# kidusabe1/Imagined-Speech-Decoding

Hardware: AMD Instinct MI355X
Metric: trials/sec end-to-end (filterbank+CNN fwd+bwd) (higher is better)
Workload: dtype f32; 1 GPU; cfg2: 64ch x 2s@256Hz EEG, 9-band Butterworth(4) filterbank -> STFT(64/32) log band power -> Conv4Layers(576,32)+Linear(32,5) fwd+bwd, softmax-CE, AdamW; trials_per_gpu=4096, global_batch=4096, parallelism=dp1, streams=one stream

## Files before the change

imagined-speech-decoding_amd/csrc/conv.hip:

```cpp
#include "common.h"
#include <math.h>
#include <string.h>
#include <type_traits>
#include <vector>

namespace isd {

typedef float f32x2 __attribute__((ext_vector_type(2)));

constexpr int kTaps = 5;
constexpr int kCK = 32;
constexpr int kMaxZones = 64;

struct ZoneDesc {
  int cin;
  int idx_off;
  int64_t p_off;
  int64_t eff_off;
  int64_t wg_off;
};

struct bf16_t { unsigned short v; };
__device__ __forceinline__ float bf16_round(float x) {
  unsigned int u = __float_as_uint(x);
// ... 2609 lines not shown
    for (int ii = wave; ii < n_it; ii += 4) {
      float* dst = buf + ii * item_len;
      glds_copy16((const float*)a.dout + ((is + ii) * a.Z + z) * (int64_t)do_len, dst, do_len >> 2, lane);
      glds_copy16((const float*)a.in + ((is + ii) * a.Ctot + chan0 + c_base) * (int64_t)a.Tx, dst + do_len,
                  (cw * a.Tin) >> 2, lane);
    }
  };
  const unsigned smem_base = (unsigned)(uintptr_t)(__attribute__((address_space(3))) float*)smem;
  const int do_q = do_len >> 2, in_q = (cw * a.Tin) >> 2;
  const bool fast = a.IPS <= 4 && do_q <= kGldsRunMax4 && in_q <= kGldsRunMax4;
  const uint64_t do_tail = __builtin_amdgcn_ballot_w64(lane < (do_q & 63));
  const uint64_t in_tail = __builtin_amdgcn_ballot_w64(lane < (in_q & 63));
  const char* do_src = (const char*)a.dout + ((i_lo + wave_s) * a.Z + z) * (int64_t)do_len * 4;
  const char* in_src = (const char*)a.in + ((i_lo + wave_s) * a.Ctot + chan0 + c_base) * (int64_t)a.Tx * 4;
  const int64_t do_step = (int64_t)a.IPS * a.Z * do_len * 4, in_step = (int64_t)a.IPS * a.Ctot * a.Tx * 4;
  const unsigned slot_lds = smem_base + (unsigned)(wave_s * item_len) * 4;
  const unsigned lane16 = lane * 16;
  auto stage_fast = [&](int n_it, int s) {
    if (wave_s < n_it) {
      const unsigned dst = slot_lds + (unsigned)(s * buf_len) * 4;
      glds_run(do_q >> 6, do_tail, dst, do_src, lane16);
      glds_run(in_q >> 6, in_tail, dst + (unsigned)do_len * 4, in_src, lane16);
    }
    do_src += do_step;
    in_src += in_step;
  };

  f32x4 acc[GT][kTaps], accb[GT];
#pragma unroll
  for (int g = 0; g < GT; ++g) {
    accb[g] = (f32x4){0.f, 0.f, 0.f, 0.f};
#pragma unroll
    for (int k = 0; k < kTaps; ++k) acc[g][k] = (f32x4){0.f, 0.f, 0.f, 0.f};
  }
  struct Frag {
    float af[GT];
    float bf[kTaps];
    float one;
  };
  const int a_off = jl * a.Tout + q;
  const int b_off = do_len + (wave * 16 + jl) * a.Tin + q;
  struct FragSet {
    float af[GT];
    f32x2 b01, b23;
    float b4;
  };
  constexpr int kSetReads = GT + 3;
  const unsigned zero_addr = smem_base + (unsigned)(2 * buf_len) * 4;
  auto run_packed = [&](auto bias, int sbuf, int n_it) {
    const unsigned buf_addr = smem_base + (unsigned)(sbuf * buf_len) * 4;
    unsigned a0 = buf_addr + (unsigned)a_off * 4, a1 = a0 + (unsigned)(16 * a.Tout) * 4, b = buf_addr + (unsigned)b_off * 4;
    int p_ii = 0, p_t = q;
    const unsigned wrap = (unsigned)(item_len - a.Tout + 4) * 4;
    auto issue = [&](FragSet& f) {
      const bool dead = p_ii >= n_it;
      const unsigned ra0 = dead ? zero_addr : a0, ra1 = dead ? zero_addr : a1, rb = dead ? zero_addr : b;
      if constexpr (GT == 2)
        asm volatile("ds_read_b32 %0, %5\n\tds_read_b32 %1, %6\n\tds_read2_b32 %2, %7 offset1:1\n\t"
                     "ds_read2_b32 %3, %7 offset0:2 offset1:3\n\tds_read_b32 %4, %7 offset:16"
                     : "=&v"(f.af[0]), "=&v"(f.af[GT - 1]), "=&v"(f.b01), "=&v"(f.b23), "=&v"(f.b4)
                     : "v"(ra0), "v"(ra1), "v"(rb)
                     : "memory");
      else
        asm volatile("ds_read_b32 %0, %4\n\tds_read2_b32 %1, %5 offset1:1\n\t"
                     "ds_read2_b32 %2, %5 offset0:2 offset1:3\n\tds_read_b32 %3, %5 offset:16"
                     : "=&v"(f.af[0]), "=&v"(f.b01), "=&v"(f.b23), "=&v"(f.b4)
                     : "v"(ra0), "v"(rb)
                     : "memory");
      p_t += 4;
      const bool w = p_t >= a.Tout;
      const unsigned d = w ? wrap : 16u;
      a0 += d; a1 += d; b += d;
      if (w) { p_t -= a.Tout; ++p_ii; }
    };
    auto take = [&](FragSet& f, auto behind) {
      if constexpr (GT == 2)
        asm volatile("s_waitcnt lgkmcnt(%5)" : "+v"(f.af[0]), "+v"(f.af[GT - 1]), "+v"(f.b01), "+v"(f.b23), "+v"(f.b4)
                     : "i"(decltype(behind)::value) : "memory");
      else
        asm volatile("s_waitcnt lgkmcnt(%4)" : "+v"(f.af[0]), "+v"(f.b01), "+v"(f.b23), "+v"(f.b4)
                     : "i"(decltype(behind)::value) : "memory");
      __builtin_amdgcn_sched_barrier(0);
    };
    auto mma_set = [&](const FragSet& f) {
      const float bf[kTaps] = {f.b01[0], f.b01[1], f.b23[0], f.b23[1], f.b4};
#pragma unroll
      for (int k = 0; k < kTaps; ++k)
#pragma unroll
        for (int g = 0; g < GT; ++g) acc[g][k] = __builtin_amdgcn_mfma_f32_16x16x4f32(f.af[g], bf[k], acc[g][k], 0, 0, 0);
      if constexpr (decltype(bias)::value) {
#pragma unroll
        for (int g = 0; g < GT; ++g) accb[g] = __builtin_amdgcn_mfma_f32_16x16x4f32(f.af[g], 1.f, accb[g], 0, 0, 0);
      }
      __builtin_amdgcn_sched_barrier(0);
    };
    const int n_step = (n_it * a.Tout + 3) >> 2;
    const std::integral_constant<int, kSetReads> one_set;
    const std::integral_constant<int, 0> none;
    FragSet f0, f1;
    issue(f0);
    int st = 1;
    for (; st + 1 < n_step; st += 2) {
      issue(f1);
      take(f0, one_set);
      mma_set(f0);
      issue(f0);
      take(f1, one_set);
      mma_set(f1);
    }
    if (st < n_step) {
      issue(f1);
      take(f0, one_set);
      mma_set(f0);
      take(f1, none);
      mma_set(f1);
    } else {
      take(f0, none);
      mma_set(f0);
    }
  };
  auto run_single = [&](int sbuf, int n_it) {
    const float* buf = smem + sbuf * buf_len;
    auto load = [&](int ii, Frag& f) {
      const bool ok = q < a.Tout;
      const float* ib = buf + ii * item_len;
#pragma unroll
      for (int g = 0; g < GT; ++g) {
        const float v = ib[a_off + g * 16 * a.Tout];
        f.af[g] = ok ? v : 0.f;
      }
#pragma unroll
      for (int k = 0; k < kTaps; ++k) {
        const float v = ib[b_off + k];
        f.bf[k] = ok ? v : 0.f;
      }
      f.one = ok ? 1.f : 0.f;
    };
    auto mma = [&](const Frag& f) {
#pragma unroll
      for (int k = 0; k < kTaps; ++k)
#pragma unroll
        for (int g = 0; g < GT; ++g) acc[g][k] = __builtin_amdgcn_mfma_f32_16x16x4f32(f.af[g], f.bf[k], acc[g][k], 0, 0, 0);
      if (with_bias) {
#pragma unroll
        for (int g = 0; g < GT; ++g) accb[g] = __builtin_amdgcn_mfma_f32_16x16x4f32(f.af[g], f.one, accb[g], 0, 0, 0);
      }
    };
    Frag f0, f1;
    load(0, f0);
    for (int st = 0; st < n_it; st += 2) {
      if (st + 1 < n_it) load(st + 1, f1);
      mma(f0);
      if (st + 1 < n_it) {
// ... 172 lines not shown

static int conv5_wgrad_wide_bf16_item_floats(int F, int W) { return (16 * F / 2 + 64 * W + 3) & ~3; }

struct ReduceDst {
  float *o0, *o1, *o2;
  int64_t n0, n1;
};
__global__ __launch_bounds__(256) void reduce_slabs_kernel(float* __restrict__ part, ReduceDst out,
                                                           int64_t n, int n_slabs, int L, int stride) {
  __shared__ float red[4][64];
  const int lane = threadIdx.x & 63, grp = threadIdx.x >> 6;
  const int64_t e = (int64_t)blockIdx.x * 64 + lane;
  const int k0 = blockIdx.y * L;
  const int k1 = k0 + L < n_slabs ? k0 + L : n_slabs;
  float s0 = 0.f, s1 = 0.f;
  if (e < n) {
    int k = k0 + grp;
    for (; k + 4 < k1; k += 8) {
      s0 += part[(int64_t)k * stride * n + e];
      s1 += part[(int64_t)(k + 4) * stride * n + e];
    }
    if (k < k1) s0 += part[(int64_t)k * stride * n + e];
  }
  red[grp][lane] = s0 + s1;
  __syncthreads();
  if (grp == 0 && e < n) {
    const float v = (red[0][lane] + red[1][lane]) + (red[2][lane] + red[3][lane]);
    if (gridDim.y > 1) part[(int64_t)k0 * stride * n + e] = v;
    else if (e < out.n0) out.o0[e] = v;
    else if (e < out.n0 + out.n1) out.o1[e - out.n0] = v;
    else out.o2[e - out.n0 - out.n1] = v;
  }
}

static inline void launch_reduce_slabs(float* part, ReduceDst out, int64_t n, int n_slabs, hipStream_t st) {
  const unsigned bx = (unsigned)cdiv(n, 64);
  if (n_slabs >= 64 && bx < 1024) {
    int L = 8;
    while (L * L < n_slabs) L *= 2;
    const int S = (int)cdiv(n_slabs, L);
    hipLaunchKernelGGL(reduce_slabs_kernel, dim3(bx, S), dim3(256), 0, st, part, out, n, n_slabs, L, 1);
    hipLaunchKernelGGL(reduce_slabs_kernel, dim3(bx, 1), dim3(256), 0, st, part, out, n, S, S, L);
  } else {
    hipLaunchKernelGGL(reduce_slabs_kernel, dim3(bx, 1), dim3(256), 0, st, part, out, n, n_slabs, n_slabs, 1);
  }
}
static inline void launch_reduce_slabs(float* part, float* out, int64_t n, int n_slabs, hipStream_t st) {
  launch_reduce_slabs(part, ReduceDst{out, nullptr, nullptr, n, 0}, n, n_slabs, st);
}

struct SlabJob {
  float* part;
  float* out;
  int64_t n;
  int n_slabs, L;
  int layer;
  unsigned bx0;
};
struct SlabJobs {
  SlabJob j[3];
  const ZoneDesc* zones;
  int F;
};
__global__ __launch_bounds__(256) void reduce_jobs_kernel(SlabJobs js, int level) {
  __shared__ float red[4][64];
  const int ji = blockIdx.x >= js.j[2].bx0 ? 2 : (blockIdx.x >= js.j[1].bx0 ? 1 : 0);
  const SlabJob jb = js.j[ji];
  const int lane = threadIdx.x & 63, grp = threadIdx.x >> 6;
  const int64_t e = (int64_t)(blockIdx.x - jb.bx0) * 64 + lane, n = jb.n;
  const int two = jb.L < jb.n_slabs;
  int k0, k1, stride;
  if (level == 2) {
    if (!two) return;
    k0 = 0; k1 = (jb.n_slabs + jb.L - 1) / jb.L; stride = jb.L;
  } else {
    k0 = blockIdx.y * jb.L;
    if (k0 >= jb.n_slabs) return;
    k1 = k0 + jb.L < jb.n_slabs ? k0 + jb.L : jb.n_slabs; stride = 1;
  }
  float s0 = 0.f, s1 = 0.f;
  if (e < n) {
    int k = k0 + grp;
    for (; k + 4 < k1; k += 8) {
      s0 += jb.part[(int64_t)k * stride * n + e];
      s1 += jb.part[(int64_t)(k + 4) * stride * n + e];
    }
    if (k < k1) s0 += jb.part[(int64_t)k * stride * n + e];
  }
  red[grp][lane] = s0 + s1;
  __syncthreads();
  if (grp == 0 && e < n) {
    const float v = (red[0][lane] + red[1][lane]) + (red[2][lane] + red[3][lane]);
    if (level == 1 && two) {
      jb.part[(int64_t)k0 * n + e] = v;
    } else if (jb.layer < 0) {
      jb.out[e] = v;
    } else {
      const int nz = js.F * js.F * kTaps;
      const int z = (int)(e / nz);
      const ZoneDesc zd = js.zones[z];
      jb.out[zd.p_off + js.F * kTaps + js.F + (int64_t)js.F * js.F * zd.cin + (int64_t)jb.layer * nz + (e - (int64_t)z * nz)] = v;
    }
  }
}

static inline int launch_reduce_fused_bwd(float* part4, float* part3, float* part0, int64_t n34, int n_slabs34, int64_t n0,
                                          int n_slabs0, float* dparams, float* wg0, const ZoneDesc* zones, int F,
                                          hipStream_t st) {
  SlabJobs js = {};
  js.zones = zones; js.F = F;
  const int64_t ns[3] = {n34, n34, n0};
  const int slabs[3] = {n_slabs34, n_slabs34, n_slabs0};
  float* parts[3] = {part4, part3, part0};
  unsigned bx = 0;
  int s_max = 1;
  bool two = false;
  for (int i = 0; i < 3; ++i) {
    SlabJob& j = js.j[i];
    j.part = parts[i]; j.n = ns[i]; j.n_slabs = slabs[i]; j.bx0 = bx;
    j.layer = i == 0 ? 1 : (i == 1 ? 0 : -1);
    j.out = i == 2 ? wg0 : dparams;
    const unsigned b = (unsigned)cdiv(ns[i], 64);
    j.L = slabs[i];
    if (slabs[i] >= 64 && b < 1024) {
      int L = 8;
      while (L * L < slabs[i]) L *= 2;
      j.L = L;
      const int S = (int)cdiv(slabs[i], L);
      if (S > s_max) s_max = S;
      two = true;
    }
    bx += b;
  }
  hipLaunchKernelGGL(reduce_jobs_kernel, dim3(bx, s_max), dim3(256), 0, st, js, two ? 1 : 0);
  if (two) hipLaunchKernelGGL(reduce_jobs_kernel, dim3(bx, 1), dim3(256), 0, st, js, 2);
  ISD_LAUNCH_CHECK();
  return ISD_OK;
}

template <int kFbwThreads>
__global__ __launch_bounds__(kFbwThreads) void fused_bwd_kernel(const float* __restrict__ params,
                                                                const ZoneDesc* __restrict__ zones,
                                                                const float* __restrict__ dweff,
                                                                float* __restrict__ dparams, int F, int nb2) {
  __shared__ float red[kFbwThreads];
  const ZoneDesc zd = zones[blockIdx.y];
  const int cz = zd.cin, cin1 = cz + 1;
  const float* W1 = params + zd.p_off;
  const float* b1 = W1 + F * kTaps;
  const float* W2 = b1 + F;
  const float* dWe = dweff + zd.wg_off;
  float* dW1 = dparams + zd.p_off;
  float* db1 = dW1 + F * kTaps;
  float* dW2 = db1 + F;
  const int blk = blockIdx.x;
  if (blk < nb2) {
    const int e = blk * kFbwThreads + threadIdx.x;
    if (e >= F * F * cz) return;
    const int c = e % cz, f = (e / cz) % F, g = e / (cz * F);
    float s = dWe[(g * cin1 + cz) * kTaps] * b1[f];
#pragma unroll
    for (int k = 0; k < kTaps; ++k) s = fmaf(dWe[(g * cin1 + c) * kTaps + k], W1[f * kTaps + k], s);
    dW2[e] = s;
    return;
  }
  const int o = blk - nb2;
  if (o >= F * kTaps + F) return;
  float s = 0.f;
  const int n_pair = F * cz;
  if (o < F * kTaps) {
    const int f = o / kTaps, k = o - f * kTaps;
#pragma unroll 4
    for (int pi = threadIdx.x; pi < n_pair; pi += kFbwThreads) {
      const int g = pi / cz, c = pi - g * cz;
      s = fmaf(dWe[(g * cin1 + c) * kTaps + k], W2[((int64_t)g * F + f) * cz + c], s);
    }
  } else {
    const int f = o - F * kTaps;
#pragma unroll 4
    for (int pi = threadIdx.x; pi < n_pair; pi += kFbwThreads) {
      const int g = pi / cz, c = pi - g * cz;
      s = fmaf(dWe[(g * cin1 + cz) * kTaps], W2[((int64_t)g * F + f) * cz + c], s);
    }
  }
  red[threadIdx.x] = s;
  __syncthreads();
  for (int w = kFbwThreads / 2; w > 0; w >>= 1) {
    if (threadIdx.x < w) red[threadIdx.x] += red[threadIdx.x + w];
    __syncthreads();
  }
// ... 71 lines not shown
  p->dma_ok = p->contiguous && (c_total % 4 == 0);
  for (int z = 0; z < n_zones; ++z)
    if (zone_sizes[z] % 4 != 0 || idx[zd[z].idx_off] % 4 != 0) p->dma_ok = 0;
  p->conv_zstride = (int64_t)(F / 4) * kTaps * GT * 64;
  hipError_t e = hipMalloc(&p->d_zones, sizeof(ZoneDesc) * n_zones);
  if (e == hipSuccess) e = hipMalloc(&p->d_idx, sizeof(int) * idx.size());
  if (e == hipSuccess) e = hipMemcpy(p->d_zones, zd.data(), sizeof(ZoneDesc) * n_zones, hipMemcpyHostToDevice);
  if (e == hipSuccess) e = hipMemcpy(p->d_idx, idx.data(), sizeof(int) * idx.size(), hipMemcpyHostToDevice);
  if (e != hipSuccess) {
    set_error("isd_conv4_plan_create: %s", hipGetErrorString(e));
    isd_conv4_plan_destroy(p);
    return e == hipErrorNoDevice ? ISD_ERR_NO_DEVICE : ISD_ERR_HIP;
  }
  *out = p;
  return ISD_OK;
}

extern "C" int isd_conv4_plan_destroy(isd_conv4_plan* p) {
  if (!p) return ISD_OK;
  if (p->d_zones) (void)hipFree(p->d_zones);
  if (p->d_idx) (void)hipFree(p->d_idx);
  delete p;
  return ISD_OK;
}

extern "C" int isd_conv4_plan_set_activation_dtype(isd_conv4_plan* p, int dtype) {
  ISD_CHECK_ARG(p && (dtype == ISD_ACT_F32 || dtype == ISD_ACT_BF16), "isd_conv4_plan_set_activation_dtype: bad argument");
  p->act_bf16 = dtype == ISD_ACT_BF16;
  return ISD_OK;
}

extern "C" int64_t isd_conv4_param_count(const isd_conv4_plan* p) { return p ? p->n_params : ISD_ERR_INVALID; }

extern "C" int64_t isd_conv4_param_offset(const isd_conv4_plan* p, int zone, int which) {
  if (!p || zone < 0 || zone >= p->Z || which < 0 || which > 4 || (which > 2 && p->n_layers != 4)) return ISD_ERR_INVALID;
  const int64_t F = p->F;
  const int64_t offs[5] = {0, F * kTaps, F * kTaps + F, F * kTaps + F + F * F * p->cz[zone],
                           F * kTaps + F + F * F * p->cz[zone] + F * F * kTaps};
  return p->p_off[zone] + offs[which];
}

extern "C" int isd_conv4_windows(const isd_conv4_plan* p, int64_t T) {
  if (!p || T < p->W) return ISD_ERR_INVALID;
  return (int)((T - p->W) / p->S + 1);
}

namespace {
enum class Route { kLayerwise, kFusedF32, kFusedBf16 };
constexpr int kFusedNW = 8;

struct Geo {
  int N, T1, TT, IPW, RS_a, RS_b, lin0, CK;
  int64_t items, act;
  int64_t o_eff, o_eff16, o_beff, o_w3, o_w3t, o_w4, o_w4t, o_a2, o_a3, o_a4, o_s, o_wg, o_wg34, o_part, total;
  int ipw0, ipw1, ns0, ns1, cw0, cw1, grp0, grp1;
  int64_t slab0, slab1;
  Route route = Route::kLayerwise;
  int fwd_per_zone = 0, bwd_per_zone = 0;
  size_t fwd_lds = 0, bwd_lds = 0;
  bool keep_dgelu = false;
  bool prep16 = false;
};

int row_stride_fwd(int need) {
  if (need <= 32) return need | 1;
  int rs = need;
  while (rs % 32 != 16) ++rs;
  return rs;
}

int per_zone_workgroups(const isd_conv4_plan* p, const Geo& g, int per_gpu) {
  int per_zone = per_gpu / p->Z;
  if (per_zone < 1) per_zone = 1;
  if (per_zone > g.items) per_zone = (int)g.items;
  return per_zone;
}

int choose_route(const isd_conv4_plan* p, Geo& g) {
  const int F = p->F;
  const size_t bwd16 = conv4_fused_bwd_bf16_lds(g.TT);
  if (p->n_layers == 4 && F == 32 && p->act_bf16 && p->max_cz <= 16 && g.TT <= 16 && g.TT >= 4 && bwd16 <= 160 * 1024) {
    g.route = Route::kFusedBf16;
    g.fwd_lds = conv4_fused_fwd_bf16_lds(g.TT);
    g.bwd_lds = bwd16;
    g.fwd_per_zone = per_zone_workgroups(p, g, g.fwd_lds <= 80 * 1024 ? 512 : 256);
    g.bwd_per_zone = per_zone_workgroups(p, g, 256);
    g.keep_dgelu = g.prep16 = true;
  } else if (p->n_layers == 4 && F == 32 && !p->act_bf16 && p->max_cz <= 16 && g.TT <= 16 && (F * g.T1) % 4 == 0 &&
             g.TT >= 4) {
    g.route = Route::kFusedF32;
    g.fwd_lds = conv4_fused_fwd_lds(kFusedNW, F, p->W, g.T1);
    g.bwd_lds = conv4_fused_bwd_lds(F, p->W, g.T1);
    ISD_CHECK_ARG(g.fwd_lds <= 150 * 1024 && g.bwd_lds <= 160 * 1024,
                  "conv4: the fused fp32 kernels need %zu / %zu bytes of LDS at window_len=%d", g.fwd_lds, g.bwd_lds, p->W);
    g.fwd_per_zone = g.bwd_per_zone = per_zone_workgroups(p, g, 256);
    g.keep_dgelu = true;
  }
  return ISD_OK;
}

int make_geo(const isd_conv4_plan* p, int64_t B, int64_t T, Geo& g) {
  ISD_CHECK_ARG(T >= p->W, "conv4: T=%lld shorter than window_len=%d", (long long)T, p->W);
  g.N = (int)((T - p->W) / p->S + 1);
  g.T1 = p->W - (kTaps - 1);
  g.TT = (g.T1 + 15) / 16;
  g.IPW = g.TT >= 16 ? 1 : 16 / g.TT;
  g.items = B * g.N;
  g.act = g.items * p->Z * p->F * g.T1;
  g.lin0 = (p->contiguous && g.N == 1 && T == p->W) ? 1 : 0;
  g.RS_a = g.lin0 ? p->W : row_stride_fwd(p->W);
  g.RS_b = g.T1;
  {
    const int GTf = p->F / 16;
    const int64_t row = g.RS_a > g.RS_b ? g.RS_a : g.RS_b;
    g.CK = kCK;
    int64_t fit = (64 * 1024 / 4 - (int64_t)(g.CK / 4) * kTaps * GTf * 64) / (g.CK * row);
    if (fit < 1) {
      while (g.CK > 4 && (150 * 1024 / 4 - 64 - (int64_t)(g.CK / 4) * kTaps * GTf * 64) / (g.CK * row) < 1) g.CK -= 4;
      fit = (150 * 1024 / 4 - 64 - (int64_t)(g.CK / 4) * kTaps * GTf * 64) / (g.CK * row);
    }
    ISD_CHECK_ARG(fit >= 1, "conv4: window_len=%d is too long for the LDS tile (about 9000 samples)", p->W);
    if (g.IPW > fit) g.IPW = (int)fit;
    const int64_t occ = (g.items * p->Z) / 512;
    int min_ipw = (4 + g.TT - 1) / g.TT;
    if (min_ipw < 1) min_ipw = 1;
    int64_t want = occ < min_ipw ? min_ipw : occ;
    if (g.IPW > want) g.IPW = (int)want;
  }
  int64_t o = 0;
  g.o_eff = o;  o += align_up(p->eff_size, 64);
  g.o_eff16 = o; o += align_up(p->eff_size / kTaps * 4, 64);
  g.o_beff = o; o += align_up((int64_t)p->Z * p->F, 64);
  const int64_t cw = align_up(p->conv_zstride * p->Z, 64);
  g.o_w3 = o; o += cw; g.o_w3t = o; o += cw; g.o_w4 = o; o += cw; g.o_w4t = o; o += cw;
  g.o_a2 = o; o += align_up(g.act, 64);
  g.o_a3 = o; o += align_up(g.act, 64);
  g.o_a4 = o; o += align_up(g.act, 64);
  g.o_s = o;  o += align_up(g.act, 64);
  g.o_wg = o; o += align_up(p->wg_size, 64);
  g.slab1 = (int64_t)p->Z * p->F * p->F * kTaps;
  g.o_wg34 = o; o += align_up(g.slab1, 64);
  auto plan_wg = [&](int cin_max, int& cw, int& ipw, int& ns, int& grp) {
    cw = cin_max >= 64 ? 64 : (int)align_up(cin_max, 16);
    grp = 4 / (cw / 16);
    const int zg = (cin_max + cw - 1) / cw;
    int64_t want = 1024 / ((int64_t)p->Z * zg);
    if (want < 1) want = 1;
    const int64_t it = g.items > 0 ? g.items : 1;
    if (want > it) want = it;
    ipw = (int)cdiv(it, want);
    ns = (int)cdiv(it, ipw) * grp;
  };
  plan_wg(p->max_cz + 1, g.cw0, g.ipw0, g.ns0, g.grp0);
  plan_wg(p->F, g.cw1, g.ipw1, g.ns1, g.grp1);
  g.slab0 = p->wg_size;
  const int64_t pa = (int64_t)g.ns0 * g.slab0, pb = (p->n_layers == 4) ? (int64_t)g.ns1 * g.slab1 : 0;
  const int64_t rz = 256 / p->Z > 1 ? 256 / p->Z : 1;
  const int64_t pf = (p->n_layers == 4) ? rz * (8 * g.slab1 + 8 * g.slab0) : 0;
  const int64_t pmax = pa > pb ? pa : pb;
  g.o_part = o; o += align_up(pmax > pf ? pmax : pf, 64);
  g.total = o;
  return choose_route(p, g);
}

template <typename Args>
void fill_geometry(Args& a, const isd_conv4_plan* p, const Geo& g, int64_t T) {
  a.zones = p->d_zones; a.chan_idx = p->d_idx; a.items = g.items; a.Z = p->Z;
  a.Ctot = p->Ctot; a.Tx = (int)T; a.N = g.N; a.S = p->S;
}
template <typename Args>
void fill_fused_geometry(Args& a, const isd_conv4_plan* p, const Geo& g, int64_t T) {
  fill_geometry(a, p, g, T);
  a.wz_stride = p->conv_zstride; a.W = p->W; a.T1 = g.T1; a.TT = g.TT;
}
ConvArgs make_conv_args(const isd_conv4_plan* p, const Geo& g, int64_t T) {
  ConvArgs a = {};
  fill_geometry(a, p, g, T);
  a.F = p->F; a.TT = g.TT; a.IPW = g.IPW; a.Tout = g.T1; a.CK = g.CK;
  return a;
}
WgradArgs make_wgrad_args(const isd_conv4_plan* p, const Geo& g, int64_t T, float* ws) {
  WgradArgs w = {};
  fill_geometry(w, p, g, T);
  w.F = p->F; w.Tout = g.T1; w.part = ws + g.o_part;
  return w;
}
FusedFwdArgs make_fused_fwd_args(const isd_conv4_plan* p, const Geo& g, const float* x, float* feat, float* ws, int64_t T) {
  FusedFwdArgs fa = {};
  fill_fused_geometry(fa, p, g, T);
  fa.x = x; fa.weff = ws + g.o_eff; fa.beff = ws + g.o_beff; fa.w3 = ws + g.o_w3; fa.w4 = ws + g.o_w4;
  fa.a2 = ws + g.o_a2; fa.a3 = ws + g.o_a3; fa.a4 = ws + g.o_a4; fa.feat = feat;
  fa.store = g.keep_dgelu ? 2 : 1;
  return fa;
}
FusedBwdArgs make_fused_bwd_args(const isd_conv4_plan* p, const Geo& g, const float* x, const float* dfeat, float* ws,
                                 int64_t T) {
  FusedBwdArgs fb = {};
  fill_fused_geometry(fb, p, g, T);
  fb.x = x; fb.dfeat = dfeat; fb.a2 = ws + g.o_a2; fb.a3 = ws + g.o_a3; fb.a4 = ws + g.o_a4;
  fb.w3t = ws + g.o_w3t; fb.w4t = ws + g.o_w4t;
  fb.part4 = ws + g.o_part;
  fb.part3 = fb.part4 + (int64_t)g.bwd_per_zone * 4 * g.slab1;
  fb.part0 = fb.part3 + (int64_t)g.bwd_per_zone * 4 * g.slab1;
  fb.slab1 = g.slab1; fb.slab0 = g.slab0;
  return fb;
}
}

extern "C" int64_t isd_conv4_workspace_bytes(const isd_conv4_plan* p, int64_t B, int64_t T) {
  if (!p || B < 0) return ISD_ERR_INVALID;
  Geo g;
  if (make_geo(p, B, T, g)) return ISD_ERR_INVALID;
  return g.total * 4;
// ... 143 lines not shown
static void (*conv5_wgrad_instance(int F))(WgradArgs) {
  return F == 32 ? conv5_wgrad_kernel<MODE, AT, true> : conv5_wgrad_kernel<MODE, AT, false>;
}

static int launch_wgrad(int mode, int bf16, WgradArgs a, int n_zones, int cin_max, hipStream_t st) {
  int64_t per_item = conv5_wgrad_item_floats(a.F, a.RSo, a.CW, a.RSi);
  int ips = (int)((96 * 1024 / 4 - 4) / per_item);
  if (ips < 1) ips = (int)((150 * 1024 / 4 - 4) / per_item);
  a.seg_len = 0;
  if (ips < 1) {
    int seg = (int)((150 * 1024 / 4 - 64 - (int64_t)a.CW * (kTaps - 1)) / (a.F + a.CW)) & ~3;
    ISD_CHECK_ARG(seg >= 16, "conv4 wgrad: no LDS segment fits");
    a.seg_len = seg;
    a.RSo = seg;
    a.RSi = seg + kTaps - 1;
    a.lin = 0;
    per_item = conv5_wgrad_item_floats(a.F, a.RSo, a.CW, a.RSi);
    ips = 1;
  }
  if (ips > 1 && per_item * 4 > 32 * 1024) ips = 1;
  const int ips_occ = (int)((32 * 1024 / 4) / per_item);
  if (ips_occ >= 1 && ips > ips_occ) ips = ips_occ;
  if (ips > 16) ips = 16;
  if (ips > a.items_per_wg) ips = a.items_per_wg;
  a.IPS = ips;
  const int64_t wgs = cdiv(a.items, a.items_per_wg);
  const int zgroups = (cin_max + a.CW - 1) / a.CW;
  void (*k)(WgradArgs);
  if (mode == 0) k = bf16 ? conv5_wgrad_instance<0, bf16_t>(a.F) : conv5_wgrad_instance<0, float>(a.F);
  else k = bf16 ? conv5_wgrad_instance<1, bf16_t>(a.F) : conv5_wgrad_instance<1, float>(a.F);
  return launch_lds(k, dim3((unsigned)wgs, n_zones, zgroups), dim3(256), conv5_wgrad_lds(ips, per_item), st, a);
}

__global__ void scatter_conv_grad_kernel(const float* __restrict__ wg, const isd::ZoneDesc* __restrict__ zones,
                                         float* __restrict__ dparams, int F, int layer) {
  const int z = blockIdx.y;
  const isd::ZoneDesc zd = zones[z];
  const int n = F * F * isd::kTaps;
  float* dst = dparams + zd.p_off + F * isd::kTaps + F + (int64_t)F * F * zd.cin + (int64_t)layer * n;
  for (int e = blockIdx.x * blockDim.x + threadIdx.x; e < n; e += gridDim.x * blockDim.x) dst[e] = wg[(int64_t)z * n + e];
}

static int launch_dweff_chain(const isd_conv4_plan* p, const float* params, const float* dweff, float* dparams,
                              hipStream_t st) {
  const int F = p->F;
  const int threads = p->max_cz >= 64 ? 1024 : 256;
  const int nb2 = (int)cdiv((int64_t)F * F * p->max_cz, threads);
  return launch_lds(threads == 1024 ? fused_bwd_kernel<1024> : fused_bwd_kernel<256>, dim3(nb2 + F * kTaps + F, p->Z),
                    dim3(threads), 0, st, params, p->d_zones, dweff, dparams, F, nb2);
}

static int first_layer_backward(const isd_conv4_plan* p, const Geo& g, const float* x, int64_t T, const float* params,
                                const float* g2, float* dparams, float* ws, hipStream_t st, bool tap16 = false,
                                bool in16 = false) {
  const int F = p->F;
  int rc;
  WgradArgs w = make_wgrad_args(p, g, T, ws);
  w.dout = g2; w.in = x; w.Tin = p->W; w.pad = 0;
  w.RSo = g.T1; w.lin = g.lin0;
  w.RSi = g.lin0 ? p->W : (p->W | 1);
  w.slab_size = g.slab0; w.wz_stride = 0; w.items_per_wg = g.ipw0; w.CW = g.cw0;
  int n_slabs0 = g.ns0;
  const int zg = (p->max_cz + 63) / 64;
  int64_t r_target = (256 * 3) / ((int64_t)zg * p->Z);
  if (r_target < 1) r_target = 1;
  if (r_target > g.ns0) r_target = g.ns0;
  const int ipw = (int)cdiv(g.items, r_target);
  const int R = (int)cdiv(g.items, ipw);
  const dim3 grid((unsigned)R, p->Z, zg);
  const int item_len = conv5_wgrad_wide_item_floats(F, g.T1, p->W);
  int ips = 4;
  while (ips > 1 && conv5_wgrad_wide_lds(ips, item_len) > 48 * 1024) --ips;
  const size_t lds = conv5_wgrad_wide_lds(ips, item_len);
  if (tap16) {
    const int ips16 = 4;
    w.items_per_wg = ipw; w.IPS = ips16;
    rc = launch_lds(in16 ? conv5_wgrad_wide_bf16_kernel<2, true> : conv5_wgrad_wide_bf16_kernel<2, false>, grid, dim3(256),
                    conv5_wgrad_wide_lds(ips16, conv5_wgrad_wide_bf16_item_floats(F, p->W)), st, w);
    n_slabs0 = R;
    g_first_wgrad_path = 2;
  } else if (g.lin0 && p->dma_ok && !p->act_bf16 && p->max_cz >= 64 && (F * g.T1) % 4 == 0 && lds <= 64 * 1024 &&
             ((uintptr_t)x & 15) == 0 && ((uintptr_t)g2 & 15) == 0) {
    w.items_per_wg = ipw; w.IPS = ips;
    rc = launch_lds(F == 32 ? conv5_wgrad_wide_kernel<2> : conv5_wgrad_wide_kernel<1>, grid, dim3(256), lds, st, w);
    n_slabs0 = R;
    g_first_wgrad_path = 1;
  } else {
    g_first_wgrad_path = 0;
    rc = launch_wgrad(0, p->act_bf16, w, p->Z, p->max_cz + 1, st);
  }
  if (rc) return rc;
  launch_reduce_slabs(ws + g.o_part, ws + g.o_wg, g.slab0, n_slabs0, st);
  return launch_dweff_chain(p, params, ws + g.o_wg, dparams, st);
}

static bool featcnn_ok(const isd_conv4_plan* p, const Geo& g, int n_cls, const void* x = nullptr) {
  return p->Z == 1 && p->n_layers == 4 && p->F == 32 && (!p->act_bf16 || bf16_mfma_ok(p, g, x)) && g.TT == 1 &&
         g.N == 1 && n_cls >= 1 && n_cls <= kTailMaxCls;
}

extern "C" int isd_featcnn_supported(const isd_conv4_plan* p, int64_t B, int64_t T, int n_cls) {
  if (!p || B < 1) return 0;
  Geo g;
  if (make_geo(p, B, T, g)) return 0;
  return featcnn_ok(p, g, n_cls) ? 1 : 0;
}

static int featcnn_step_impl(const isd_conv4_plan* p, const float* x, const float* params, const float* fc_w,
                             const float* fc_b, const void* labels, int label_bytes, float* dparams, float* dfc,
                             float* logits, int64_t* pred, float* loss, void* workspace, int64_t B, int64_t T,
                             int n_cls, float grad_scale, void* stream, bool x_bf16) {
  ISD_CHECK_ARG(p, "isd_featcnn_step: null plan");
  ISD_CHECK_ARG(B >= 1, "isd_featcnn_step: B=%lld", (long long)B);
  Geo g;
  int rc = make_geo(p, B, T, g);
  if (rc) return rc;
  if (!featcnn_ok(p, g, n_cls, x)) {
    set_error("isd_featcnn_step: needs one zone, 4 layers, 32 filters, <= 16 output steps (bf16 activations: <= 13, over "
              "whole 16-byte aligned rows of at most 17 samples), <= %d classes", kTailMaxCls);
    return ISD_ERR_UNSUPPORTED;
  }
  const bool tap16 = p->act_bf16 != 0;
  if (x_bf16 && !(tap16 && p->max_cz % 8 == 0)) {
    set_error("isd_featcnn_step_bf16: a bf16 feature map needs a plan with bf16 activations and a multiple of 8 input "
              "channels (got act_bf16=%d, %d channels)", p->act_bf16, p->max_cz);
    return ISD_ERR_UNSUPPORTED;
  }
  ISD_CHECK_ARG(x && params && fc_w && fc_b && logits && pred && workspace, "isd_featcnn_step: null argument");
  ISD_CHECK_ARG(!labels || label_bytes == 1 || label_bytes == 8, "isd_featcnn_step: labels must be uint8 or int64");
  const bool train = labels && dparams && dfc;
  ISD_CHECK_ARG(!labels || loss, "isd_featcnn_step: labels without a loss pointer");
  hipStream_t st = (hipStream_t)stream;
  float* ws = (float*)workspace;
  const int F = p->F;
  rc = launch_prep(p, g, params, ws, st, tap16);
  if (rc) return rc;
  ConvArgs a = {};
  rc = first_layer_forward(p, g, x, T, ws, st, a, tap16, x_bf16);
  if (rc) return rc;
  TailArgs t = {};
  t.a2 = ws + g.o_a2; t.g2 = ws + g.o_a4;
  t.w3 = ws + g.o_w3; t.w4 = ws + g.o_w4; t.w3t = ws + g.o_w3t; t.w4t = ws + g.o_w4t;
  t.fc_w = fc_w; t.fc_b = fc_b; t.labels = labels; t.label_bytes = label_bytes;
  t.logits = logits; t.pred = pred; t.part = ws + g.o_part;
  t.items = g.items; t.T1 = g.T1; t.n_cls = n_cls; t.train = train ? 1 : 0; t.grad_scale = grad_scale;
  const int n34 = 2 * F * F * kTaps, nfc = n_cls * (F + 1);
  t.slab = n34 + nfc + 1;
  auto tail_blocks = [&](int items_per_wg) {
    const int64_t b = cdiv(g.items, items_per_wg);
    return b > 256 ? 256 : b < 1 ? 1 : (int)b;
  };
  constexpr int TNW = 8;
  constexpr int BNW = 8;
  int blocks = tail_blocks(TNW);
  size_t lds = featcnn_tail_lds(TNW, F);
  ISD_CHECK_ARG(lds <= 160 * 1024 && (int64_t)blocks * t.slab <= g.total - g.o_part, "isd_featcnn_step: workspace");
  if (tap16) {
    blocks = tail_blocks(BNW * 2);
    lds = featcnn_tail_bf16_lds(BNW, F);
    ISD_CHECK_ARG(lds <= 160 * 1024 && (int64_t)blocks * t.slab <= g.total - g.o_part, "isd_featcnn_step: workspace");
    rc = launch_lds(featcnn_tail_bf16_kernel<BNW>, dim3(blocks), dim3(BNW * 64), lds, st, t);
  } else {
    rc = launch_lds(featcnn_tail_kernel<TNW>, dim3(blocks), dim3(TNW * 64), lds, st, t);
  }
  if (rc) return rc;
  if (!labels) return ISD_OK;
  if (train) {
    float* dw34 = dparams + p->p_off[0] + F * kTaps + F + (int64_t)F * F * p->cz[0];
    launch_reduce_slabs(ws + g.o_part, ReduceDst{dw34, dfc, loss, n34, nfc}, t.slab, blocks, st);
  } else {
    float* red = ws + g.o_s;
    launch_reduce_slabs(ws + g.o_part, ReduceDst{red, red + n34, loss, n34, nfc}, t.slab, blocks, st);
  }
  ISD_LAUNCH_CHECK();
  if (!train) return ISD_OK;
  return first_layer_backward(p, g, x, T, params, ws + g.o_a4, dparams, ws, st, tap16, x_bf16);
}

extern "C" int isd_featcnn_step(const isd_conv4_plan* p, const float* x, const float* params, const float* fc_w,
                                const float* fc_b, const void* labels, int label_bytes, float* dparams, float* dfc,
                                float* logits, int64_t* pred, float* loss, void* workspace, int64_t B, int64_t T,
                                int n_cls, float grad_scale, void* stream) {
  return featcnn_step_impl(p, x, params, fc_w, fc_b, labels, label_bytes, dparams, dfc, logits, pred, loss, workspace, B,
                           T, n_cls, grad_scale, stream, false);
}

extern "C" int isd_featcnn_step_bf16(const isd_conv4_plan* p, const uint16_t* x, const float* params, const float* fc_w,
                                     const float* fc_b, const void* labels, int label_bytes, float* dparams, float* dfc,
                                     float* logits, int64_t* pred, float* loss, void* workspace, int64_t B, int64_t T,
                                     int n_cls, float grad_scale, void* stream) {
  return featcnn_step_impl(p, reinterpret_cast<const float*>(x), params, fc_w, fc_b, labels, label_bytes, dparams, dfc,
                           logits, pred, loss, workspace, B, T, n_cls, grad_scale, stream, true);
}

static int launch_fused_backward(void (*kernel)(FusedBwdArgs), int slabs34, int slabs0, const isd_conv4_plan* p,
                                 const Geo& g, const FusedBwdArgs& fb, const float* params, float* dparams, float* ws,
                                 hipStream_t st) {
  int rc = launch_lds(kernel, dim3(g.bwd_per_zone, p->Z), dim3(kFusedNW * 64), g.bwd_lds, st, fb);
  if (rc) return rc;
  rc = launch_reduce_fused_bwd(fb.part4, fb.part3, fb.part0, g.slab1, g.bwd_per_zone * slabs34, g.slab0,
                               g.bwd_per_zone * slabs0, dparams, ws + g.o_wg, p->d_zones, p->F, st);
  if (rc) return rc;
  return launch_dweff_chain(p, params, ws + g.o_wg, dparams, st);
}

static int fused_backward(const isd_conv4_plan* p, const Geo& g, const float* x, const float* params, const float* dfeat,
                          float* dparams, float* ws, int64_t T, hipStream_t st) {
  const FusedBwdArgs fb = make_fused_bwd_args(p, g, x, dfeat, ws, T);
  if (g.route == Route::kFusedBf16)
    return launch_fused_backward(conv4_fused_bwd_bf16_kernel<kFusedNW>, 4, kFusedNW, p, g, fb, params, dparams, ws, st);
  return launch_fused_backward(conv4_fused_bwd_kernel<kFusedNW>, 2, 4, p, g, fb, params, dparams, ws, st);
}

static int launch_gelu_mean_bwd(const isd_conv4_plan* p, const Geo& g, float* top, const float* dfeat, bool pre,
                                hipStream_t st) {
  const int64_t rows = g.items * p->Z * p->F;
  void (*k)(void*, const float*, int64_t, int) = gelu_mean_bwd_kernel<bf16_t>;
  if (!p->act_bf16) k = pre ? gelu_mean_bwd_kernel<float, true> : gelu_mean_bwd_kernel<float>;
  return launch_lds(k, dim3((unsigned)cdiv(rows * 16, 256)), dim3(256), 0, st, top, dfeat, rows, g.T1);
}

static int conv4_backward_impl(const isd_conv4_plan* p, const float* x, const float* params, const float* dfeat,
                               float* dparams, float* dx, void* workspace, int64_t B, int64_t T, void* stream) {
  ISD_CHECK_ARG(p, "isd_conv4_backward: null plan");
  ISD_CHECK_ARG(B >= 0, "isd_conv4_backward: B=%lld", (long long)B);
  Geo g;
  int rc = make_geo(p, B, T, g);
  if (rc) return rc;
  ISD_CHECK_ARG(dparams, "isd_conv4_backward: null dparams");
// ... 66 lines not shown
```

Before: 3.949 million trials/s.

## Defer tail slab reduction into first-layer wgrad reduce launch and fence first LDS set

The feature-CNN tail's gradient partials now go to a dedicated workspace region, so their slab reduction no longer has to run before the first-layer backward reuses the shared partial buffer. That reduction is merged with the layer-0 wgrad reduction into one job-based reduce launch, which saves kernel launches. The generic job reducer is extended with split destinations and reordered so two-level jobs go first. Separately, the first LDS fragment issue in the packed conv loop adds a conditional full lgkmcnt wait when only one step runs. The cost is extra workspace and more complex reducer indexing.

Measured after the change: 3.942 million trials/s. About the same (-0.2%).

```diff
diff --git a/imagined-speech-decoding_amd/csrc/conv.hip b/imagined-speech-decoding_amd/csrc/conv.hip
--- a/imagined-speech-decoding_amd/csrc/conv.hip
+++ b/imagined-speech-decoding_amd/csrc/conv.hip
@@ -2685,27 +2685,44 @@
     unsigned a0 = buf_addr + (unsigned)a_off * 4, a1 = a0 + (unsigned)(16 * a.Tout) * 4, b = buf_addr + (unsigned)b_off * 4;
     int p_ii = 0, p_t = q;
     const unsigned wrap = (unsigned)(item_len - a.Tout + 4) * 4;
-    auto issue = [&](FragSet& f) {
+    const int n_step = (n_it * a.Tout + 3) >> 2;
+    auto issue_set = [&](FragSet& f, auto first) {
       const bool dead = p_ii >= n_it;
       const unsigned ra0 = dead ? zero_addr : a0, ra1 = dead ? zero_addr : a1, rb = dead ? zero_addr : b;
-      if constexpr (GT == 2)
+      if constexpr (GT == 2 && !decltype(first)::value)
         asm volatile("ds_read_b32 %0, %5\n\tds_read_b32 %1, %6\n\tds_read2_b32 %2, %7 offset1:1\n\t"
                      "ds_read2_b32 %3, %7 offset0:2 offset1:3\n\tds_read_b32 %4, %7 offset:16"
                      : "=&v"(f.af[0]), "=&v"(f.af[GT - 1]), "=&v"(f.b01), "=&v"(f.b23), "=&v"(f.b4)
                      : "v"(ra0), "v"(ra1), "v"(rb)
                      : "memory");
-      else
+      else if constexpr (GT == 2)
+        asm volatile("ds_read_b32 %0, %5\n\tds_read_b32 %1, %6\n\tds_read2_b32 %2, %7 offset1:1\n\t"
+                     "ds_read2_b32 %3, %7 offset0:2 offset1:3\n\tds_read_b32 %4, %7 offset:16\n\t"
+                     "s_cmp_lg_u32 %8, 1\n\ts_cbranch_scc1 1f\n\ts_waitcnt lgkmcnt(0)\n1:"
+                     : "=&v"(f.af[0]), "=&v"(f.af[GT - 1]), "=&v"(f.b01), "=&v"(f.b23), "=&v"(f.b4)
+                     : "v"(ra0), "v"(ra1), "v"(rb), "s"(n_step)
+                     : "memory", "scc");
+      else if constexpr (!decltype(first)::value)
         asm volatile("ds_read_b32 %0, %4\n\tds_read2_b32 %1, %5 offset1:1\n\t"
                      "ds_read2_b32 %2, %5 offset0:2 offset1:3\n\tds_read_b32 %3, %5 offset:16"
                      : "=&v"(f.af[0]), "=&v"(f.b01), "=&v"(f.b23), "=&v"(f.b4)
                      : "v"(ra0), "v"(rb)
                      : "memory");
+      else
+        asm volatile("ds_read_b32 %0, %4\n\tds_read2_b32 %1, %5 offset1:1\n\t"
+                     "ds_read2_b32 %2, %5 offset0:2 offset1:3\n\tds_read_b32 %3, %5 offset:16\n\t"
+                     "s_cmp_lg_u32 %6, 1\n\ts_cbranch_scc1 1f\n\ts_waitcnt lgkmcnt(0)\n1:"
+                     : "=&v"(f.af[0]), "=&v"(f.b01), "=&v"(f.b23), "=&v"(f.b4)
+                     : "v"(ra0), "v"(rb), "s"(n_step)
+                     : "memory", "scc");
       p_t += 4;
       const bool w = p_t >= a.Tout;
       const unsigned d = w ? wrap : 16u;
       a0 += d; a1 += d; b += d;
       if (w) { p_t -= a.Tout; ++p_ii; }
     };
+    auto issue = [&](FragSet& f) { issue_set(f, std::false_type{}); };
+    auto issue_first = [&](FragSet& f) { issue_set(f, std::true_type{}); };
     auto take = [&](FragSet& f, auto behind) {
       if constexpr (GT == 2)
         asm volatile("s_waitcnt lgkmcnt(%5)" : "+v"(f.af[0]), "+v"(f.af[GT - 1]), "+v"(f.b01), "+v"(f.b23), "+v"(f.b4)
@@ -2727,11 +2744,10 @@
       }
       __builtin_amdgcn_sched_barrier(0);
     };
-    const int n_step = (n_it * a.Tout + 3) >> 2;
     const std::integral_constant<int, kSetReads> one_set;
     const std::integral_constant<int, 0> none;
     FragSet f0, f1;
-    issue(f0);
+    issue_first(f0);
     int st = 1;
     for (; st + 1 < n_step; st += 2) {
       issue(f1);
@@ -3010,7 +3026,8 @@
 struct SlabJob {
   float* part;
   float* out;
-  int64_t n;
+  float *o1, *o2;
+  int64_t n, n0, n1;
   int n_slabs, L;
   int layer;
   unsigned bx0;
@@ -3028,10 +3045,10 @@
   const int64_t e = (int64_t)(blockIdx.x - jb.bx0) * 64 + lane, n = jb.n;
   const int two = jb.L < jb.n_slabs;
   int k0, k1, stride;
-  if (level == 2) {
-    if (!two) return;
+  if (level == 2 && two) {
     k0 = 0; k1 = (jb.n_slabs + jb.L - 1) / jb.L; stride = jb.L;
   } else {
+    if (level == 1 && !two) return;
     k0 = blockIdx.y * jb.L;
     if (k0 >= jb.n_slabs) return;
     k1 = k0 + jb.L < jb.n_slabs ? k0 + jb.L : jb.n_slabs; stride = 1;
@@ -3052,7 +3069,9 @@
     if (level == 1 && two) {
       jb.part[(int64_t)k0 * n + e] = v;
     } else if (jb.layer < 0) {
-      jb.out[e] = v;
+      if (e < jb.n0) jb.out[e] = v;
+      else if (e < jb.n0 + jb.n1) jb.o1[e - jb.n0] = v;
+      else jb.o2[e - jb.n0 - jb.n1] = v;
     } else {
       const int nz = js.F * js.F * kTaps;
       const int z = (int)(e / nz);
@@ -3062,38 +3081,53 @@
   }
 }
 
+static inline int launch_reduce_jobs(SlabJobs& js, int n_jobs, hipStream_t st) {
+  SlabJob jobs[3];
+  int n_two = 0, s_max = 1;
+  for (int pass = 0; pass < 2; ++pass)
+    for (int i = 0, o = n_two; i < n_jobs; ++i) {
+      SlabJob j = js.j[i];
+      const bool two = j.n_slabs >= 64 && cdiv(j.n, 64) < 1024;
+      if (two != (pass == 0)) continue;
+      j.L = j.n_slabs;
+      if (two) {
+        int L = 8;
+        while (L * L < j.n_slabs) L *= 2;
+        j.L = L;
+        const int S = (int)cdiv(j.n_slabs, L);
+        if (S > s_max) s_max = S;
+      }
+      jobs[pass == 0 ? n_two++ : o++] = j;
+    }
+  unsigned bx = 0, bx_two = 0;
+  for (int i = 0; i < 3; ++i) {
+    if (i < n_jobs) js.j[i] = jobs[i];
+    js.j[i].bx0 = bx;
+    if (i < n_jobs) bx += (unsigned)cdiv(js.j[i].n, 64);
+    if (i + 1 == n_two) bx_two = bx;
+  }
+  if (n_two) hipLaunchKernelGGL(reduce_jobs_kernel, dim3(bx_two, s_max), dim3(256), 0, st, js, 1);
+  hipLaunchKernelGGL(reduce_jobs_kernel, dim3(bx, 1), dim3(256), 0, st, js, n_two ? 2 : 0);
+  ISD_LAUNCH_CHECK();
+  return ISD_OK;
+}
+
+static inline SlabJob contiguous_job(float* part, ReduceDst out, int64_t n, int n_slabs) {
+  SlabJob j = {};
+  j.part = part; j.out = out.o0; j.o1 = out.o1; j.o2 = out.o2; j.n = n; j.n0 = out.n0; j.n1 = out.n1;
+  j.n_slabs = n_slabs; j.layer = -1;
+  return j;
+}
+
 static inline int launch_reduce_fused_bwd(float* part4, float* part3, float* part0, int64_t n34, int n_slabs34, int64_t n0,
                                           int n_slabs0, float* dparams, float* wg0, const ZoneDesc* zones, int F,
                                           hipStream_t st) {
   SlabJobs js = {};
   js.zones = zones; js.F = F;
-  const int64_t ns[3] = {n34, n34, n0};
-  const int slabs[3] = {n_slabs34, n_slabs34, n_slabs0};
-  float* parts[3] = {part4, part3, part0};
-  unsigned bx = 0;
-  int s_max = 1;
-  bool two = false;
-  for (int i = 0; i < 3; ++i) {
-    SlabJob& j = js.j[i];
-    j.part = parts[i]; j.n = ns[i]; j.n_slabs = slabs[i]; j.bx0 = bx;
-    j.layer = i == 0 ? 1 : (i == 1 ? 0 : -1);
-    j.out = i == 2 ? wg0 : dparams;
-    const unsigned b = (unsigned)cdiv(ns[i], 64);
-    j.L = slabs[i];
-    if (slabs[i] >= 64 && b < 1024) {
-      int L = 8;
-      while (L * L < slabs[i]) L *= 2;
-      j.L = L;
-      const int S = (int)cdiv(slabs[i], L);
-      if (S > s_max) s_max = S;
-      two = true;
-    }
-    bx += b;
-  }
-  hipLaunchKernelGGL(reduce_jobs_kernel, dim3(bx, s_max), dim3(256), 0, st, js, two ? 1 : 0);
-  if (two) hipLaunchKernelGGL(reduce_jobs_kernel, dim3(bx, 1), dim3(256), 0, st, js, 2);
-  ISD_LAUNCH_CHECK();
-  return ISD_OK;
+  js.j[0].part = part4; js.j[0].out = dparams; js.j[0].n = n34; js.j[0].n_slabs = n_slabs34; js.j[0].layer = 1;
+  js.j[1].part = part3; js.j[1].out = dparams; js.j[1].n = n34; js.j[1].n_slabs = n_slabs34; js.j[1].layer = 0;
+  js.j[2] = contiguous_job(part0, ReduceDst{wg0, nullptr, nullptr, n0, 0}, n0, n_slabs0);
+  return launch_reduce_jobs(js, 3, st);
 }
 
 template <int kFbwThreads>
@@ -3271,7 +3305,7 @@
 struct Geo {
   int N, T1, TT, IPW, RS_a, RS_b, lin0, CK;
   int64_t items, act;
-  int64_t o_eff, o_eff16, o_beff, o_w3, o_w3t, o_w4, o_w4t, o_a2, o_a3, o_a4, o_s, o_wg, o_wg34, o_part, total;
+  int64_t o_eff, o_eff16, o_beff, o_w3, o_w3t, o_w4, o_w4t, o_a2, o_a3, o_a4, o_s, o_wg, o_wg34, o_part, o_tail, tail_len, total;
   int ipw0, ipw1, ns0, ns1, cw0, cw1, grp0, grp1;
   int64_t slab0, slab1;
   Route route = Route::kLayerwise;
@@ -3378,6 +3412,10 @@
   const int64_t pf = (p->n_layers == 4) ? rz * (8 * g.slab1 + 8 * g.slab0) : 0;
   const int64_t pmax = pa > pb ? pa : pb;
   g.o_part = o; o += align_up(pmax > pf ? pmax : pf, 64);
+  g.tail_len = 0;
+  if (p->Z == 1 && p->n_layers == 4 && g.TT == 1 && g.N == 1)
+    g.tail_len = 256 * ((int64_t)2 * p->F * p->F * kTaps + (int64_t)kTailMaxCls * (p->F + 1) + 1);
+  g.o_tail = o; o += align_up(g.tail_len, 64);
   g.total = o;
   return choose_route(p, g);
 }
@@ -3627,7 +3665,7 @@
 
 static int first_layer_backward(const isd_conv4_plan* p, const Geo& g, const float* x, int64_t T, const float* params,
                                 const float* g2, float* dparams, float* ws, hipStream_t st, bool tap16 = false,
-                                bool in16 = false) {
+                                bool in16 = false, const SlabJob* tail = nullptr) {
   const int F = p->F;
   int rc;
   WgradArgs w = make_wgrad_args(p, g, T, ws);
@@ -3665,7 +3703,15 @@
     rc = launch_wgrad(0, p->act_bf16, w, p->Z, p->max_cz + 1, st);
   }
   if (rc) return rc;
-  launch_reduce_slabs(ws + g.o_part, ws + g.o_wg, g.slab0, n_slabs0, st);
+  if (tail) {
+    SlabJobs js = {};
+    js.j[0] = *tail;
+    js.j[1] = contiguous_job(ws + g.o_part, ReduceDst{ws + g.o_wg, nullptr, nullptr, g.slab0, 0}, g.slab0, n_slabs0);
+    rc = launch_reduce_jobs(js, 2, st);
+    if (rc) return rc;
+  } else {
+    launch_reduce_slabs(ws + g.o_part, ws + g.o_wg, g.slab0, n_slabs0, st);
+  }
   return launch_dweff_chain(p, params, ws + g.o_wg, dparams, st);
 }
 
@@ -3717,7 +3763,7 @@
   t.a2 = ws + g.o_a2; t.g2 = ws + g.o_a4;
   t.w3 = ws + g.o_w3; t.w4 = ws + g.o_w4; t.w3t = ws + g.o_w3t; t.w4t = ws + g.o_w4t;
   t.fc_w = fc_w; t.fc_b = fc_b; t.labels = labels; t.label_bytes = label_bytes;
-  t.logits = logits; t.pred = pred; t.part = ws + g.o_part;
+  t.logits = logits; t.pred = pred; t.part = ws + g.o_tail;
   t.items = g.items; t.T1 = g.T1; t.n_cls = n_cls; t.train = train ? 1 : 0; t.grad_scale = grad_scale;
   const int n34 = 2 * F * F * kTaps, nfc = n_cls * (F + 1);
   t.slab = n34 + nfc + 1;
@@ -3729,27 +3775,26 @@
   constexpr int BNW = 8;
   int blocks = tail_blocks(TNW);
   size_t lds = featcnn_tail_lds(TNW, F);
-  ISD_CHECK_ARG(lds <= 160 * 1024 && (int64_t)blocks * t.slab <= g.total - g.o_part, "isd_featcnn_step: workspace");
+  ISD_CHECK_ARG(lds <= 160 * 1024 && (int64_t)blocks * t.slab <= g.tail_len, "isd_featcnn_step: workspace");
   if (tap16) {
     blocks = tail_blocks(BNW * 2);
     lds = featcnn_tail_bf16_lds(BNW, F);
-    ISD_CHECK_ARG(lds <= 160 * 1024 && (int64_t)blocks * t.slab <= g.total - g.o_part, "isd_featcnn_step: workspace");
+    ISD_CHECK_ARG(lds <= 160 * 1024 && (int64_t)blocks * t.slab <= g.tail_len, "isd_featcnn_step: workspace");
     rc = launch_lds(featcnn_tail_bf16_kernel<BNW>, dim3(blocks), dim3(BNW * 64), lds, st, t);
   } else {
     rc = launch_lds(featcnn_tail_kernel<TNW>, dim3(blocks), dim3(TNW * 64), lds, st, t);
   }
   if (rc) return rc;
   if (!labels) return ISD_OK;
-  if (train) {
-    float* dw34 = dparams + p->p_off[0] + F * kTaps + F + (int64_t)F * F * p->cz[0];
-    launch_reduce_slabs(ws + g.o_part, ReduceDst{dw34, dfc, loss, n34, nfc}, t.slab, blocks, st);
-  } else {
+  if (!train) {
     float* red = ws + g.o_s;
-    launch_reduce_slabs(ws + g.o_part, ReduceDst{red, red + n34, loss, n34, nfc}, t.slab, blocks, st);
-  }
-  ISD_LAUNCH_CHECK();
-  if (!train) return ISD_OK;
-  return first_layer_backward(p, g, x, T, params, ws + g.o_a4, dparams, ws, st, tap16, x_bf16);
+    launch_reduce_slabs(ws + g.o_tail, ReduceDst{red, red + n34, loss, n34, nfc}, t.slab, blocks, st);
+    ISD_LAUNCH_CHECK();
+    return ISD_OK;
+  }
+  float* dw34 = dparams + p->p_off[0] + F * kTaps + F + (int64_t)F * F * p->cz[0];
+  const SlabJob tail = contiguous_job(ws + g.o_tail, ReduceDst{dw34, dfc, loss, n34, nfc}, t.slab, blocks);
+  return first_layer_backward(p, g, x, T, params, ws + g.o_a4, dparams, ws, st, tap16, x_bf16, &tail);
 }
 
 extern "C" int isd_featcnn_step(const isd_conv4_plan* p, const float* x, const float* params, const float* fc_w,
```
